# dcy0577/Enhancing-3D-Point-Cloud-Segmentation-Using-Multi-Modal-Fusion-with-2D-Images

Measured on AMD Instinct MI355X. Metric: input points/s through MV-KPConv KPFCNN forward+backward (pyramid + fusion + fwd + bwd + SGD), higher is better.
Workload: dtype f32; 1 GPU; early_fusion_kpfcnn5_sphere19k_x1_per_gpu; views=3, parallelism=dp1, execution=hipGraph[net|chain|enc2d(x2 every 2nd step)+fa], ranks=1, input_lookahead_batches=2, capacity_overflow=False

## Files before the change

enhancing-3d-point-cloud-segmentation-using-multi-modal-fusion-with-2d-images_amd/csrc/gemm.hip:

```cpp
#include <stdlib.h>

#include <mutex>
#include <type_traits>

#include "common.h"

namespace {

typedef float f32x4 __attribute__((ext_vector_type(4)));

constexpr int BK = 32;

template <bool CONTIG_K, int ROWS>
struct Tile {
  static constexpr int LD = CONTIG_K ? 40 : ROWS + 4;
  static constexpr int FLOATS = CONTIG_K ? ROWS * 40 : BK * (ROWS + 4);
  static constexpr int NF4 = ROWS * BK / 4;
  static constexpr int NV = (NF4 + 255) / 256;
  static constexpr int IPT = ROWS / 4;
  float4 v[NV];

  __device__ __forceinline__ void transform(const float* __restrict__ xs, int64_t k0, int64_t kbase0, int64_t i0, int64_t imax,
                                            int64_t kmax, int64_t nvalid, float slope, float* __restrict__ out, int64_t ld,
                                            int tid) {
    static_assert(CONTIG_K, "the transform is written for k-contiguous A tiles");
#pragma unroll
    for (int u = 0; u < NV; ++u) {
      const int f = tid + 256 * u;
      if (NF4 % 256 == 0 || f < NF4) {
        const int i = f >> 3, kq = (f & 7) * 4;
        const int64_t gi = i0 + i, gk = k0 + kq;
        const float* t = xs + (gk - kbase0) * 4;
        float e[4] = {v[u].x, v[u].y, v[u].z, v[u].w};
#pragma unroll
        for (int c = 0; c < 4; ++c) {
          const float4 q = *reinterpret_cast<const float4*>(t + 4 * c);
          float z = (e[c] - q.x) * q.y + q.z;
          z = z > 0.f ? z : z * slope;
          e[c] = gi < nvalid ? z : 0.f;
        }
        v[u] = make_float4(e[0], e[1], e[2], e[3]);
        if (out && gi < imax) {
          float* o = out + gi * ld + gk;
          if (gk + 3 < kmax && (ld & 3) == 0)
            *reinterpret_cast<float4*>(o) = v[u];
          else {
#pragma unroll
            for (int c = 0; c < 4; ++c)
              if (gk + c < kmax) o[c] = e[c];
// ... 67 lines not shown
        const int k = f / IPT, iq = (f % IPT) * 4;
        int64_t gi = i0 + iq;
        gi = gi + 3 < imax ? gi : imax - 4;
        p = src + (k0 + k) * ld + gi;
      }
      if (VEC == 4) {
        const f32x4 q = *reinterpret_cast<const f32x4*>(p);
        v[u] = make_float4(q[0], q[1], q[2], q[3]);
      } else {
        const float2 q0 = *reinterpret_cast<const float2*>(p), q1 = *reinterpret_cast<const float2*>(p + 2);
        v[u] = make_float4(q0.x, q0.y, q1.x, q1.y);
      }
    }
  }

  static __device__ __forceinline__ bool fast_ok(int64_t imax, int vec) {
    return CONTIG_K ? (vec >= 2 && imax >= 1) : (vec == 4 && imax >= 4 && (imax & 3) == 0);
  }

  template <int VEC>
  __device__ __forceinline__ void fetch(const float* __restrict__ src, int64_t ld, int64_t i0, int64_t imax, int64_t k0,
                                        int64_t kmax, int vec, int tid) {
    if (VEC == 0)
      load(src, ld, i0, imax, k0, kmax, vec, tid);
    else
      load_fast<VEC>(src, ld, i0, imax, k0, tid);
  }

  __device__ __forceinline__ void store(float* __restrict__ T, int tid) const {
#pragma unroll
    for (int u = 0; u < NV; ++u) {
      const int f = tid + 256 * u;
      if (NF4 % 256 == 0 || f < NF4) {
        const f32x4 q = {v[u].x, v[u].y, v[u].z, v[u].w};
        if (CONTIG_K) {
          const int i = f >> 3, kq = (f & 7) * 4;
          *reinterpret_cast<f32x4*>(&T[i * LD + kq]) = q;
        } else {
          const int k = f / IPT, iq = (f % IPT) * 4;
          *reinterpret_cast<f32x4*>(&T[k * LD + iq]) = q;
        }
      }
    }
  }

  static __device__ __forceinline__ f32x4 frag(const float* __restrict__ T, int r0, int j, int lane) {
    const int i = lane & 15, g = lane >> 4;
    if (CONTIG_K) {
      return *reinterpret_cast<const f32x4*>(&T[(r0 + i) * LD + 16 * j + 4 * g]);
    } else {
      f32x4 r;
      const float* p = &T[(16 * j + 4 * g) * LD + r0 + i];
      r[0] = p[0];
      r[1] = p[LD];
      r[2] = p[2 * LD];
      r[3] = p[3 * LD];
      return r;
    }
  }
};

struct GemmArgs {
  const float* A;
  const float* B;
  float* C;
  int64_t M, N, Kd, lda, ldb, k_per_split;
  int atomic_out, accumulate, vecA, vecB;
  float* bn_part;
  const int32_t* n_valid;
  const float* bias;
  float act_slope;
  const float* A2;
  const float* B2;
  int64_t Kd2, lda2, ldb2;
  int vecA2, vecB2;
  const void* sc_idx;
  int sc_idx64, sc_c1;
  int64_t sc_stride, sc_ns;
  float* sc_dst;
  float* sc_rest;
  float* det_ws;
  int* det_cnt;
  int det_gx, det_nsplit;
  int seg_shift;
  int64_t seg_extra;
  int* fin_cnt;
  int fin_gy;
  float fin_eps, fin_momentum;
  float* fin_mean;
  float* fin_invstd;
  float* fin_rmean;
  float* fin_rvar;
  long long* fin_nbt;
  const float* ax_mean;
  const float* ax_invstd;
  const float* ax_gamma;
  const float* ax_beta;
  float ax_slope;
  const int32_t* ax_nvalid;
  float* ax_out;
};

constexpr int XF_KMAX = 512;

template <bool TA, bool TB, int PM, int QN, int WM, int WN, bool DUAL = false, bool XF = false>
__device__ __forceinline__ void gemm_body(const GemmArgs& a, const int bx, const int by, const int bz) {
  static_assert(WM * WN == 4, "four waves per workgroup");
  constexpr int TM = 16 * PM * WM, TN = 16 * QN * WN;
  typedef Tile<!TA, TM> TileA;
  typedef Tile<TB, TN> TileB;
  __shared__ __attribute__((aligned(16))) float lds[2 * (TileA::FLOATS + TileB::FLOATS)];
  __shared__ __attribute__((aligned(16))) float xs[XF ? 4 * (XF_KMAX + BK) : 4];
  float* const As = lds;
  float* const Bs = lds + 2 * TileA::FLOATS;
  const int tid = threadIdx.x, lane = tid & 63, wave = tid >> 6;
  const int wm = wave / WN, wn = wave % WN;
  const int64_t m0 = (int64_t)by * TM, n0 = (int64_t)bx * TN;
  const int64_t ktot = DUAL ? a.Kd + a.Kd2 : a.Kd;
  const int64_t kbeg_all = (int64_t)bz * a.k_per_split;
  const int64_t kend_all = kbeg_all + a.k_per_split < ktot ? kbeg_all + a.k_per_split : ktot;

  f32x4 acc[PM][QN];
#pragma unroll
  for (int p = 0; p < PM; ++p)
#pragma unroll
    for (int q = 0; q < QN; ++q) acc[p][q] = (f32x4){0.f, 0.f, 0.f, 0.f};

  int64_t x_nvalid = 0;
  if (XF) {
    for (int k = tid; k < XF_KMAX + BK; k += 256) {
      const int64_t gk = kbeg_all + k;
      float4 q = make_float4(0.f, 0.f, 0.f, 0.f);
      if (gk < a.Kd && k < a.k_per_split + BK) q = make_float4(a.ax_mean[gk], a.ax_invstd[gk] * a.ax_gamma[gk], a.ax_beta[gk], 0.f);
      *reinterpret_cast<float4*>(&xs[4 * k]) = q;
    }
    x_nvalid = a.ax_nvalid ? (int64_t)*a.ax_nvalid : a.M;
    __syncthreads();
  }
  float* const x_out = (XF && bx == 0) ? a.ax_out : nullptr;

  TileA la0, la1;
  TileB lb0, lb1;
  const int ra = wm * 16 * PM, rb = wn * 16 * QN;
  auto compute = [&](const float* __restrict__ Ta, const float* __restrict__ Tb) {
#pragma unroll
    for (int j = 0; j < 2; ++j) {
      f32x4 fa[PM], fb[QN];
#pragma unroll
      for (int p = 0; p < PM; ++p) fa[p] = TileA::frag(Ta, ra + 16 * p, j, lane);
#pragma unroll
      for (int q = 0; q < QN; ++q) fb[q] = TileB::frag(Tb, rb + 16 * q, j, lane);
#pragma unroll
      for (int s = 0; s < 4; ++s)
#pragma unroll
        for (int p = 0; p < PM; ++p)
#pragma unroll
          for (int q = 0; q < QN; ++q)
            acc[p][q] = __builtin_amdgcn_mfma_f32_16x16x4f32(fa[p][s], fb[q][s], acc[p][q], 0, 0, 0);
    }
  };
  float* const A0 = As;
  float* const A1 = As + TileA::FLOATS;
  float* const B0 = Bs;
  float* const B1 = Bs + TileB::FLOATS;
  auto run_range = [&](const float* __restrict__ pA, const int64_t lda, const int vecA, const float* __restrict__ pB,
                       const int64_t ldb, const int vecB, int64_t kbeg, const int64_t kend) {
  auto Bat = [&](const int64_t k) -> const float* {
    return (TB && !DUAL && a.seg_shift >= 0) ? pB + (k >> a.seg_shift) * a.seg_extra : pB;
  };
  auto putA = [&](TileA& la, float* __restrict__ T, const int64_t kt) {
    if constexpr (XF) la.transform(xs, kt, kbeg_all, m0, a.M, a.Kd, x_nvalid, a.ax_slope, x_out, lda, tid);
    la.store(T, tid);
  };
  auto pipeline = [&](auto va, auto vb, const int64_t klim) {
    constexpr int VA = decltype(va)::value, VB = decltype(vb)::value;
    if (kbeg >= klim) return;
    la0.template fetch<VA>(pA, lda, m0, a.M, kbeg, klim, vecA, tid);
// ... 270 lines not shown
      float* const qr = lds + 2 * 256 * 4;
      if (bl == 0) *reinterpret_cast<f32x4*>(&qr[4 * c4]) = ref;
      __syncthreads();
      const int64_t col = n0 + tid;
      if (tid < TN && col < a.N) {
        float x = 0.f, y = 0.f;
#pragma unroll 4
        for (int l = 0; l < BL; ++l) {
          x += q1[l * TN + tid];
          y += q2[l * TN + tid];
        }
        float mu = 0.f, var = 0.f, is = 0.f;
        if (nv > 0) {
          mu = x / (float)nv;
          const float dm = mu - qr[tid];
          float M2 = y - (float)nv * dm * dm;
          M2 = M2 > 0.f ? M2 : 0.f;
          var = M2 / (float)nv;
          is = rsqrtf(var + a.fin_eps);
        }
        a.fin_mean[col] = mu;
        a.fin_invstd[col] = is;
        if (a.fin_rmean && nv > 0) {
          const float unbiased = nv > 1 ? var * ((float)nv / (float)(nv - 1)) : var;
          a.fin_rmean[col] = (1.f - a.fin_momentum) * a.fin_rmean[col] + a.fin_momentum * mu;
          a.fin_rvar[col] = (1.f - a.fin_momentum) * a.fin_rvar[col] + a.fin_momentum * unbiased;
        }
      }
      if (a.fin_nbt && bx == 0 && tid == 0) *a.fin_nbt += 1;
    }
  }
}

template <bool TA, bool TB, int PM, int QN, int WM, int WN>
__global__ __launch_bounds__(256) void gemm_f32_mfma(const GemmArgs a) {
  gemm_body<TA, TB, PM, QN, WM, WN>(a, blockIdx.x, blockIdx.y, blockIdx.z);
}

template <bool TB, int PM>
__global__ __launch_bounds__(256) void gemm_f32_mfma_xf(const GemmArgs a) {
  gemm_body<false, TB, PM, 1, 1, 4, false, true>(a, blockIdx.x, blockIdx.y, blockIdx.z);
}

template <bool TA, bool TB, int PM, int QN, int WM, int WN>
__global__ __launch_bounds__(256) void gemm_f32_mfma_pair(const GemmArgs a0, const GemmArgs a1, int gx0, int gz0, int gz1) {
  if ((int)blockIdx.x < gx0) {
    if ((int)blockIdx.z >= gz0) return;
    gemm_body<TA, TB, PM, QN, WM, WN>(a0, blockIdx.x, blockIdx.y, blockIdx.z);
  } else {
    if ((int)blockIdx.z >= gz1) return;
    gemm_body<TA, TB, PM, QN, WM, WN>(a1, blockIdx.x - gx0, blockIdx.y, blockIdx.z);
  }
}

template <bool TA, bool TB, int PM, int QN, int WM, int WN>
__global__ __launch_bounds__(256) void gemm_f32_mfma_dual(const GemmArgs a) {
  gemm_body<TA, TB, PM, QN, WM, WN, true>(a, blockIdx.x, blockIdx.y, blockIdx.z);
}

struct GroupEntry {
  GemmArgs args;
  int gx, gy, gz;
  int wg_begin;
};

template <bool TA, bool TB, int PM, int QN, int WM, int WN>
__global__ __launch_bounds__(256) void gemm_f32_mfma_grouped(const GroupEntry* __restrict__ tab, int n_prob) {
  const int b = blockIdx.x;
  int lo = 0, hi = n_prob - 1;
  while (lo < hi) {
    const int mid = (lo + hi + 1) >> 1;
    if (tab[mid].wg_begin <= b)
      lo = mid;
    else
      hi = mid - 1;
  }
  const GroupEntry& e = tab[lo];
  const int local = b - e.wg_begin;
  const int bx = local % e.gx, by = (local / e.gx) % e.gy, bz = local / (e.gx * e.gy);
  GemmArgs a = e.args;
  a.A = load_global_ptr(&e.args.A);
  a.B = load_global_ptr(&e.args.B);
  a.C = load_global_ptr(&e.args.C);
  a.bn_part = load_global_ptr(&e.args.bn_part);
  a.n_valid = load_global_ptr(&e.args.n_valid);
  a.det_ws = load_global_ptr(&e.args.det_ws);
  a.det_cnt = load_global_ptr(&e.args.det_cnt);
  gemm_body<TA, TB, PM, QN, WM, WN>(a, bx, by, bz);
}


struct Plan {
  int pm, qn, narrow, split;
};

struct SplitArena {
  float* ws = nullptr;
  int* cnt = nullptr;
  int64_t ws_floats = 0, n_cnt = 0;
  int64_t ws_off = 0, cnt_off = 0;
  int64_t ws_top = 0, cnt_top = 0;
};
SplitArena g_arena;
std::mutex g_arena_mu;

bool ordered_splits() { return g_arena.ws != nullptr; }

int arena_take(hipStream_t st, int64_t tiles, int split, int64_t slot, float** ws, int** cnt) {
  const int64_t need = (tiles * split * slot + 63) / 64 * 64;
  std::lock_guard<std::mutex> lock(g_arena_mu);
  if (need > g_arena.ws_floats || tiles > g_arena.n_cnt) return 1;
  hipStreamCaptureStatus cap = hipStreamCaptureStatusNone;
  if (hipStreamIsCapturing(st, &cap) != hipSuccess) {
    (void)hipGetLastError();
    cap = hipStreamCaptureStatusNone;
  }
  if (cap != hipStreamCaptureStatusNone) {
    if (g_arena.ws_top - need < g_arena.ws_off || g_arena.cnt_top - tiles < g_arena.cnt_off) return 2;
    g_arena.ws_top -= need;
    g_arena.cnt_top -= tiles;
    *ws = g_arena.ws + g_arena.ws_top;
    *cnt = g_arena.cnt + g_arena.cnt_top;
    return 0;
  }
  const int64_t ws_cap = g_arena.ws_top < g_arena.ws_floats / 4 ? g_arena.ws_top : (need > g_arena.ws_floats / 4 ? need : g_arena.ws_floats / 4);
  const int64_t cnt_cap = g_arena.cnt_top < g_arena.n_cnt / 4 ? g_arena.cnt_top : (tiles > g_arena.n_cnt / 4 ? tiles : g_arena.n_cnt / 4);
  if (g_arena.ws_off + need > ws_cap || g_arena.cnt_off + tiles > cnt_cap) {
// ... 1 lines not shown
    if (hipDeviceSynchronize() != hipSuccess) return -2;
    g_arena.ws_off = 0;
    g_arena.cnt_off = 0;
  }
  *ws = g_arena.ws + g_arena.ws_off;
  *cnt = g_arena.cnt + g_arena.cnt_off;
  g_arena.ws_off += need;
  g_arena.cnt_off += tiles;
  return 0;
}

const char* arena_error(int rc) {
  return rc == 1 ? "the split-reduction arena is smaller than one product's parking space (MVK_GEMM_ARENA_MB)"
         : rc == 2 ? "the split-reduction arena is used up by the slices captured graphs hold for good: too small for the "
                     "captured steps of this process (MVK_GEMM_ARENA_MB)"
                   : "hipDeviceSynchronize failed while recycling the split-reduction arena";
}

int make_ordered(hipStream_t st, GemmArgs& a, int split, int gx, int64_t gy, int64_t tm, int64_t tn) {
  a.det_ws = nullptr; a.det_cnt = nullptr; a.det_gx = gx; a.det_nsplit = split;
  if (split <= 1 || !ordered_splits()) return 0;
  const int rc = arena_take(st, (int64_t)gx * gy, split, tm * tn, &a.det_ws, &a.det_cnt);
  if (rc != 0) return rc;
  a.atomic_out = 0;
  return 0;
}

#define MVK_ORDERED(call)                                      \
  do {                                                         \
    const int _rc = (call);                                    \
    MVK_REQUIRE(_rc == 0, "gemm: %s", arena_error(_rc));       \
  } while (0)

Plan plan_gemm(int64_t M, int64_t N, int64_t Kd, int split_req, bool want_stats) {
  const int narrow = N <= 32 ? 1 : 0;
  const int pm = narrow ? 1 : (want_stats ? 4 : 2), qn = narrow ? (N <= 16 ? 1 : 2) : 1;
  const int64_t tm = narrow ? 64 * pm : 16 * pm, tn = narrow ? 16 * qn : 64 * qn;
  const int64_t tiles = cdiv64(M, tm) * cdiv64(N, tn), ksteps = cdiv64(Kd, BK);
  Plan best{pm, qn, narrow, 1};
  double best_t = 1e300, t1 = 1e300;
  for (int split = 1; split <= 64; ++split) {
    if (split_req > 0 && split != split_req) continue;
    if (split > 1 && ksteps / split < 4) break;
    const int64_t kt = cdiv64(ksteps, split), wgs = tiles * split;
    double t = (double)cdiv64(wgs, 1280) * (kt * 1500.0 + 3000.0) + (double)wgs * kt * 256.0 * pm * qn / 256.0;
    if (split > 1) t += (double)M * N * split * 4.0 / 2160.0 + 500.0 * split;
    if (split == 1) t1 = t;
    if (t < best_t) {
      best_t = t;
      best.split = split;
    }
  }
  static double bonus = -1.0;
  if (bonus < 0.0) {
    const char* eb = getenv("MVK_GEMM_STATS_BONUS");
    bonus = eb ? atof(eb) : 14000.0;
  }
  if (want_stats && !ordered_splits() && t1 <= best_t + bonus) best.split = 1;
  const char* e = getenv("MVK_GEMM_FORCE");
  if (e) {
    int pm = 0, qn = 0, sp = 0;
    if (sscanf(e, "%d,%d,%d", &pm, &qn, &sp) == 3) {
      if (pm > 0) best.pm = pm;
      if (qn > 0 && !best.narrow) best.qn = qn;
      if (sp > 0 && split_req <= 0) best.split = sp;
    }
  }
  return best;
}

template <bool TA, bool TB, int PM, int QN, int WM, int WN>
void launch_one(dim3 grid, hipStream_t st, const GemmArgs& a) {
  hipLaunchKernelGGL((gemm_f32_mfma<TA, TB, PM, QN, WM, WN>), grid, dim3(256), 0, st, a);
}

template <bool TA, bool TB>
bool launch_cfg(const Plan& p, dim3 grid, hipStream_t st, const GemmArgs& a) {
  if (p.narrow) {
#define NARROW(PMv, QNv) \
  if (p.pm == PMv && p.qn == QNv) return launch_one<TA, TB, PMv, QNv, 4, 1>(grid, st, a), true
    NARROW(1, 1); NARROW(2, 1); NARROW(1, 2); NARROW(2, 2);
#undef NARROW
    return false;
  }
#define WIDE(PMv, QNv) \
  if (p.pm == PMv && p.qn == QNv) return launch_one<TA, TB, PMv, QNv, 1, 4>(grid, st, a), true
  WIDE(1, 1); WIDE(2, 1); WIDE(4, 1); WIDE(5, 1);
  WIDE(1, 2); WIDE(2, 2); WIDE(4, 2);
#undef WIDE
  return false;
}

template <bool TA, bool TB, int PM>
void launch_pair_one(dim3 grid, hipStream_t st, const GemmArgs& a0, const GemmArgs& a1, int gx0, int gz0, int gz1) {
  hipLaunchKernelGGL((gemm_f32_mfma_pair<TA, TB, PM, 1, 1, 4>), grid, dim3(256), 0, st, a0, a1, gx0, gz0, gz1);
}

template <bool TA, bool TB>
bool launch_pair_cfg(const Plan& p, dim3 grid, hipStream_t st, const GemmArgs& a0, const GemmArgs& a1, int gx0, int gz0, int gz1) {
  if (p.qn != 1) return false;
  if (p.pm == 2) return launch_pair_one<TA, TB, 2>(grid, st, a0, a1, gx0, gz0, gz1), true;
  if (p.pm == 4) return launch_pair_one<TA, TB, 4>(grid, st, a0, a1, gx0, gz0, gz1), true;
  return false;
}

void pair_widen(Plan& a, const Plan& b, int64_t Kd) {
  if (a.narrow && !b.narrow && Kd <= 512) {
    a.narrow = 0;
    a.pm = b.pm;
    a.qn = 1;
    a.split = 1;
  }
}

void no_bn_fold(GemmArgs& a) {
  a.fin_cnt = nullptr; a.fin_gy = 0; a.fin_eps = 0.f; a.fin_momentum = 0.f; a.fin_mean = nullptr; a.fin_invstd = nullptr;
  a.fin_rmean = nullptr; a.fin_rvar = nullptr; a.fin_nbt = nullptr;
  a.ax_mean = nullptr; a.ax_invstd = nullptr; a.ax_gamma = nullptr; a.ax_beta = nullptr; a.ax_slope = 1.f;
  a.ax_nvalid = nullptr; a.ax_out = nullptr;
}

int set_finish(GemmArgs& a, const mvk_bn_finish* fin, int64_t gy) {
  if (!fin) return 0;
  MVK_REQUIRE(a.bn_part != nullptr, "gemm: finished BatchNorm statistics need the statistics epilogue (plan: stat rows 0)");
  MVK_REQUIRE(fin->counters && fin->mean && fin->invstd && a.N % 4 == 0 && (uintptr_t)a.bn_part % 16 == 0,
              "gemm: finished statistics need counters, mean, invstd and a channel count that is a multiple of 4");
  MVK_REQUIRE((fin->running_mean == nullptr) == (fin->running_var == nullptr), "gemm: running_mean and running_var go together");
  a.fin_cnt = fin->counters; a.fin_gy = (int)gy; a.fin_eps = fin->eps; a.fin_momentum = fin->momentum;
  a.fin_mean = fin->mean; a.fin_invstd = fin->invstd; a.fin_rmean = fin->running_mean; a.fin_rvar = fin->running_var;
  a.fin_nbt = (long long*)fin->num_batches_tracked;
  return 0;
}

// ... 50 lines not shown
extern "C" int mvk_gemm_split_ordered(void) { return ordered_splits() ? 1 : 0; }

extern "C" int mvk_gemm_f32_dual_plan(int64_t M, int64_t N, int64_t Kd, int64_t Kd2, int* out_split) {
  MVK_REQUIRE(M >= 0 && N >= 0 && Kd >= 0 && Kd2 >= 0 && out_split, "gemm dual plan: bad arguments");
  *out_split = 0;
  if (M == 0 || N == 0 || Kd == 0 || Kd2 == 0 || Kd % BK != 0) return 0;
  const Plan p = plan_gemm(M, N, Kd + Kd2, 0, false);
  if (p.narrow || p.qn != 1 || p.pm != 2) return 0;
  int split = p.split;
  const int64_t ksteps = cdiv64(Kd + Kd2, BK);
  if (split > ksteps) split = (int)ksteps;
  const int64_t k_per_split = cdiv64(ksteps, split) * BK;
  *out_split = (int)cdiv64(Kd + Kd2, k_per_split);
  return 0;
}

extern "C" int mvk_gemm_f32_dual(const float* A, const float* B, const float* A2, const float* B2, float* C, int64_t M,
                                 int64_t N, int64_t Kd, int64_t Kd2, void* stream) {
  MVK_REQUIRE(M > 0 && N > 0 && Kd > 0 && Kd2 > 0 && Kd % BK == 0, "gemm dual: unsupported shape (ask mvk_gemm_f32_dual_plan)");
  const Plan p = plan_gemm(M, N, Kd + Kd2, 0, false);
  MVK_REQUIRE(!p.narrow && p.qn == 1 && p.pm == 2, "gemm dual: unsupported shape (ask mvk_gemm_f32_dual_plan)");
  hipStream_t st = (hipStream_t)stream;
  GemmArgs a;
  const int split = fill_args(a, p, A, B, C, M, N, Kd + Kd2, 0, 0, nullptr, nullptr);
  a.Kd = Kd;
  a.lda = Kd;
  a.vecA = ((a.lda % 4 == 0) && ((uintptr_t)A % 16 == 0)) ? 4 : ((a.lda % 2 == 0) && ((uintptr_t)A % 8 == 0)) ? 2 : 1;
  a.A2 = A2; a.B2 = B2; a.Kd2 = Kd2; a.lda2 = Kd2; a.ldb2 = N;
  a.vecA2 = ((a.lda2 % 4 == 0) && ((uintptr_t)A2 % 16 == 0)) ? 4 : ((a.lda2 % 2 == 0) && ((uintptr_t)A2 % 8 == 0)) ? 2 : 1;
  a.vecB2 = ((a.ldb2 % 4 == 0) && ((uintptr_t)B2 % 16 == 0)) ? 4 : ((a.ldb2 % 2 == 0) && ((uintptr_t)B2 % 8 == 0)) ? 2 : 1;
  MVK_REQUIRE(cdiv64(M, 32) < 65536 && split < 65536, "gemm: grid too large");
  dim3 grid((unsigned)cdiv64(N, 64), (unsigned)cdiv64(M, 32), (unsigned)split);
  MVK_ORDERED(make_ordered(st, a, split, (int)grid.x, grid.y, 32, 64));
  hipLaunchKernelGGL((gemm_f32_mfma_dual<false, false, 2, 1, 1, 4>), grid, dim3(256), 0, st, a);
  MVK_CHECK_HIP(hipGetLastError());
  return 0;
}

extern "C" int mvk_gemm_f32_pair_plan(int64_t M, int64_t N0, int64_t N1, int64_t Kd, int want_stats, int* out ) {
  MVK_REQUIRE(M >= 0 && N0 >= 0 && N1 >= 0 && Kd >= 0 && out, "gemm pair plan: bad arguments");
  for (int i = 0; i < 5; ++i) out[i] = 0;
  if (M == 0 || N0 == 0 || N1 == 0 || Kd == 0) return 0;
  Plan p0 = plan_gemm(M, N0, Kd, 0, want_stats != 0), p1 = plan_gemm(M, N1, Kd, 0, want_stats != 0);
  pair_widen(p0, p1, Kd);
  if (p0.narrow || p1.narrow || p0.pm != p1.pm || p0.qn != 1 || p1.qn != 1 || (p0.pm != 2 && p0.pm != 4)) return 0;
  out[0] = 1;
  out[1] = p0.split;
  out[2] = p1.split;
  out[3] = (want_stats && (p0.split == 1 || ordered_splits())) ? 16 * p0.pm : 0;
  out[4] = (want_stats && (p1.split == 1 || ordered_splits())) ? 16 * p1.pm : 0;
  return 0;
}

namespace {
int gemm_pair_run(const float* A, const float* B0, const float* B1, float* C0, float* C1, int64_t M, int64_t N0, int64_t N1,
                  int64_t Kd, int transB, int want_stats, float* bn_part0, float* bn_part1, const int32_t* n_valid,
                  const mvk_bn_finish* fin0, const mvk_bn_finish* fin1, void* stream);
}
extern "C" int mvk_gemm_f32_pair(const float* A, const float* B0, const float* B1, float* C0, float* C1, int64_t M,
                                 int64_t N0, int64_t N1, int64_t Kd, int transB, int want_stats, float* bn_part0,
                                 float* bn_part1, const int32_t* n_valid, void* stream) {
  return gemm_pair_run(A, B0, B1, C0, C1, M, N0, N1, Kd, transB, want_stats, bn_part0, bn_part1, n_valid, nullptr, nullptr, stream);
}
extern "C" int mvk_gemm_f32_pair_bn(const float* A, const float* B0, const float* B1, float* C0, float* C1, int64_t M,
                                    int64_t N0, int64_t N1, int64_t Kd, int transB, float* bn_part0, float* bn_part1,
                                    const int32_t* n_valid, const mvk_bn_finish* fin0, const mvk_bn_finish* fin1, void* stream) {
  return gemm_pair_run(A, B0, B1, C0, C1, M, N0, N1, Kd, transB, 1, bn_part0, bn_part1, n_valid, fin0, fin1, stream);
}
namespace {
int gemm_pair_run(const float* A, const float* B0, const float* B1, float* C0, float* C1, int64_t M, int64_t N0, int64_t N1,
                  int64_t Kd, int transB, int want_stats, float* bn_part0, float* bn_part1, const int32_t* n_valid,
                  const mvk_bn_finish* fin0, const mvk_bn_finish* fin1, void* stream) {
  MVK_REQUIRE(M > 0 && N0 > 0 && N1 > 0 && Kd > 0, "gemm pair: empty product");
  Plan p0 = plan_gemm(M, N0, Kd, 0, want_stats != 0), p1 = plan_gemm(M, N1, Kd, 0, want_stats != 0);
  pair_widen(p0, p1, Kd);
  MVK_REQUIRE(!p0.narrow && !p1.narrow && p0.pm == p1.pm && p0.qn == 1 && p1.qn == 1 && (p0.pm == 2 || p0.pm == 4),
              "gemm pair: the two products do not share a tile shape (ask mvk_gemm_f32_pair_plan first)");
  hipStream_t st = (hipStream_t)stream;
  GemmArgs a0, a1;
  const bool ord = ordered_splits();
  const int s0 = fill_args(a0, p0, A, B0, C0, M, N0, Kd, 0, transB, (want_stats && (p0.split == 1 || ord)) ? bn_part0 : nullptr, n_valid);
  const int s1 = fill_args(a1, p1, A, B1, C1, M, N1, Kd, 0, transB, (want_stats && (p1.split == 1 || ord)) ? bn_part1 : nullptr, n_valid);
  const int64_t tm = 16 * p0.pm, tn = 64;
  MVK_REQUIRE(cdiv64(M, tm) < 65536 && s0 < 65536 && s1 < 65536, "gemm: grid too large");
  const int gx0 = (int)cdiv64(N0, tn), gx1 = (int)cdiv64(N1, tn);
  MVK_ORDERED(make_ordered(st, a0, s0, gx0, cdiv64(M, tm), tm, tn));
  MVK_ORDERED(make_ordered(st, a1, s1, gx1, cdiv64(M, tm), tm, tn));
  MVK_REQUIRE(ord || ((s0 == 1 || !a0.bn_part) && (s1 == 1 || !a1.bn_part)), "gemm pair: statistics of a split product");
  if (int e = set_finish(a0, fin0, cdiv64(M, tm))) return e;
  if (int e = set_finish(a1, fin1, cdiv64(M, tm))) return e;
  dim3 grid((unsigned)(gx0 + gx1), (unsigned)cdiv64(M, tm), (unsigned)(s0 > s1 ? s0 : s1));
  const bool ok = transB ? launch_pair_cfg<false, true>(p0, grid, st, a0, a1, gx0, s0, s1)
                         : launch_pair_cfg<false, false>(p0, grid, st, a0, a1, gx0, s0, s1);
  MVK_REQUIRE(ok, "gemm pair: no kernel for plan pm=%d", p0.pm);
  MVK_CHECK_HIP(hipGetLastError());
  return 0;
}
}

extern "C" int mvk_gemm_f32_plan(int64_t M, int64_t N, int64_t Kd, int split_k, int want_stats, int* out_split,
                                 int* out_stat_rows) {
  MVK_REQUIRE(M >= 0 && N >= 0 && Kd >= 0 && out_split && out_stat_rows, "gemm plan: bad arguments");
  if (M == 0 || N == 0 || Kd == 0) {
    *out_split = 1;
    *out_stat_rows = 0;
    return 0;
  }
  const Plan p = plan_gemm(M, N, Kd, split_k > 0 ? split_k : 0, want_stats != 0);
// ... 42 lines not shown
  while ((1 << shift) < Cout) ++shift;
  return gemm_run(A, W, dx, M, Cin, (int64_t)K * Cout, 0, 1, 0, 0, nullptr, nullptr, nullptr, 1.f, stream, nullptr, shift,
                  (int64_t)Cin * Cout - Cout);
}

extern "C" int mvk_gemm_f32_ldb(const float* A, const float* B, float* C, int64_t M, int64_t N, int64_t Kd, int64_t ldb,
                                void* stream) {
  MVK_REQUIRE(ldb >= N, "gemm ldb: ldb < N");
  return gemm_run(A, B, C, M, N, Kd, 0, 0, 0, 0, nullptr, nullptr, nullptr, 1.f, stream, nullptr, -1, 0, ldb);
}

extern "C" int mvk_gemm_f32_scatter_cat(const float* A, const float* B, int64_t M, int64_t N, int64_t Kd, const void* idx,
                                        int idx64, int64_t idx_stride, int64_t Ns, int c1, float* d_x, float* d_skip,
                                        void* stream) {
  MVK_REQUIRE(idx && d_x && d_skip && c1 > 0 && c1 < N && Kd > 0 && Ns >= 0 && idx_stride >= 1, "gemm scatter_cat: bad arguments");
  const ScatterOut sc{idx, idx64, c1, idx_stride, Ns, d_x, d_skip};
  return gemm_run(A, B, d_skip , M, N, Kd, 0, 0, 0, 0, nullptr, nullptr, nullptr, 1.f, stream, &sc);
}

namespace {
int gemm_run(const float* A, const float* B, float* C, int64_t M, int64_t N, int64_t Kd, int transA, int transB,
             int accumulate, int split_k, float* bn_part, const int32_t* n_valid, const float* bias, float act_slope,
             void* stream, const ScatterOut* scatter, int seg_shift, int64_t seg_extra, int64_t ldb,
             const mvk_bn_finish* fin, const mvk_a_transform* ax) {
  MVK_REQUIRE(M >= 0 && N >= 0 && Kd >= 0, "gemm: negative size");
  if (M == 0 || N == 0) return 0;
  hipStream_t st = (hipStream_t)stream;
  MVK_REQUIRE(!(bn_part && (accumulate || Kd == 0)), "gemm: BatchNorm statistics need a plain store of a non-empty product");
  if (Kd == 0) {
    if (!accumulate && split_k <= 1) MVK_CHECK_HIP(hipMemsetAsync(C, 0, sizeof(float) * M * N, st));
    return 0;
  }
  MVK_REQUIRE(!(bn_part && split_k > 1 && !ordered_splits()), "gemm: BatchNorm statistics need an unsplit (or ordered) reduction");
  Plan p = plan_gemm(M, N, Kd, (bn_part && !ordered_splits()) ? 1 : (split_k > 0 ? split_k : 0), bn_part != nullptr);
  int split = p.split;
  const int64_t ksteps = cdiv64(Kd, BK);
  if (split > ksteps) split = (int)ksteps;
  const int64_t k_per_split = cdiv64(ksteps, split) * BK;
  split = (int)cdiv64(Kd, k_per_split);
  GemmArgs a;
  a.A = A; a.B = B; a.C = C; a.M = M; a.N = N; a.Kd = Kd;
  a.lda = transA ? M : Kd;
  a.ldb = transB ? Kd : N;
  a.k_per_split = k_per_split;
  a.atomic_out = split > 1;
  a.accumulate = accumulate;
  a.vecA = ((a.lda % 4 == 0) && ((uintptr_t)A % 16 == 0)) ? 4 : ((a.lda % 2 == 0) && ((uintptr_t)A % 8 == 0)) ? 2 : 1;
  a.vecB = ((a.ldb % 4 == 0) && ((uintptr_t)B % 16 == 0)) ? 4 : ((a.ldb % 2 == 0) && ((uintptr_t)B % 8 == 0)) ? 2 : 1;
  if (ldb > 0) {
    a.ldb = ldb;
    a.vecB = ((a.ldb % 4 == 0) && ((uintptr_t)B % 16 == 0)) ? 4 : ((a.ldb % 2 == 0) && ((uintptr_t)B % 8 == 0)) ? 2 : 1;
  }
  if (seg_shift >= 0) {
    a.ldb = (int64_t)1 << seg_shift;
    a.vecB = ((uintptr_t)B % 16 == 0 && seg_extra % 4 == 0) ? 4 : 1;
  }
  a.bn_part = bn_part;
  a.n_valid = n_valid;
  a.bias = bias;
  a.act_slope = act_slope;
  a.A2 = nullptr; a.B2 = nullptr; a.Kd2 = 0; a.lda2 = 0; a.ldb2 = 0; a.vecA2 = 1; a.vecB2 = 1;
  a.sc_idx = nullptr; a.sc_idx64 = 0; a.sc_c1 = 0; a.sc_stride = 0; a.sc_ns = 0; a.sc_dst = nullptr; a.sc_rest = nullptr;
  a.seg_shift = seg_shift;
  a.seg_extra = seg_extra;
  no_bn_fold(a);
  if (scatter) {
    a.sc_idx = scatter->idx; a.sc_idx64 = scatter->idx64; a.sc_c1 = scatter->c1; a.sc_stride = scatter->stride;
// ... 7 lines not shown
  if (int e = set_finish(a, fin, grid.y)) return e;
  if (ax) {
    MVK_REQUIRE(!transA && transB && !p.narrow && p.qn == 1 && (p.pm == 2 || p.pm == 4) && k_per_split <= XF_KMAX && !scatter &&
                    seg_shift < 0 && ax->mean && ax->invstd && ax->gamma && ax->beta && ax->slope > 0.f,
                "gemm: the operand transform needs an NT product of more than 32 columns with k-ranges <= %d", XF_KMAX);
    a.ax_mean = ax->mean; a.ax_invstd = ax->invstd; a.ax_gamma = ax->gamma; a.ax_beta = ax->beta; a.ax_slope = ax->slope;
    a.ax_nvalid = ax->n_valid; a.ax_out = ax->out;
    if (p.pm == 2) hipLaunchKernelGGL((gemm_f32_mfma_xf<true, 2>), grid, dim3(256), 0, st, a);
    else hipLaunchKernelGGL((gemm_f32_mfma_xf<true, 4>), grid, dim3(256), 0, st, a);
    MVK_CHECK_HIP(hipGetLastError());
    return 0;
  }
  bool ok;
  if (!transA && !transB) ok = launch_cfg<false, false>(p, grid, st, a);
  else if (!transA && transB) ok = launch_cfg<false, true>(p, grid, st, a);
  else if (transA && !transB) ok = launch_cfg<true, false>(p, grid, st, a);
  else ok = launch_cfg<true, true>(p, grid, st, a);
  MVK_REQUIRE(ok, "gemm: no kernel for plan pm=%d qn=%d narrow=%d", p.pm, p.qn, p.narrow);
  MVK_CHECK_HIP(hipGetLastError());
  return 0;
}
}

struct MvkGemmProblem {
  const float* A;
  const float* B;
  float* C;
  int64_t M, N, Kd;
};

extern "C" int64_t mvk_gemm_group_entry_bytes(void) { return (int64_t)sizeof(GroupEntry); }

constexpr int GROUP_KTILES_MIN = 16, GROUP_KTILES_MAX = 96;

int group_wide_pm() {
  static const int v = getenv("MVK_DW_WIDE_PM") ? atoi(getenv("MVK_DW_WIDE_PM")) : 4;
  return v == 2 || v == 8 ? v : 4;
}

int group_ktiles_env() {
  static const int v = getenv("MVK_DW_GROUP_KTILES") ? atoi(getenv("MVK_DW_GROUP_KTILES")) : -1;
  return v;
}

int grouped_split_at(int64_t M, int64_t N, int64_t Kd, int ktiles) {
  if (ktiles <= 0) return plan_gemm(M, N, Kd, 0, false).split;
  int64_t split = cdiv64(cdiv64(Kd, BK), ktiles);
  return (int)(split > 64 ? 64 : (split < 1 ? 1 : split));
}

extern "C" int mvk_gemm_f32_tn_grouped_split(int64_t M, int64_t N, int64_t Kd) {
  const int e = group_ktiles_env();
  return grouped_split_at(M, N, Kd, e >= 0 ? e : GROUP_KTILES_MIN);
}

extern "C" int mvk_gemm_f32_tn_grouped_plan(const void* problems, int n, void* table_host, int* n_narrow,
                                            int64_t* wgs_narrow, int64_t* wgs_wide, int32_t* splits ,
                                            void* stream ) {
  MVK_REQUIRE(n >= 0 && problems && table_host && n_narrow && wgs_narrow && wgs_wide && splits, "grouped gemm: bad arguments");
  const MvkGemmProblem* pr = (const MvkGemmProblem*)problems;
  GroupEntry* tab = (GroupEntry*)table_host;
  int nn = 0;
  for (int i = 0; i < n; ++i) nn += pr[i].N <= 32 ? 1 : 0;
  int64_t wn = 0, ww = 0;
  int in = 0, iw = nn;
  int ktiles = group_ktiles_env();
// ... 31 lines not shown
    e.args.sc_idx = nullptr; e.args.sc_idx64 = 0; e.args.sc_c1 = 0; e.args.sc_stride = 0; e.args.sc_ns = 0;
    e.args.sc_dst = nullptr; e.args.sc_rest = nullptr;
    e.args.seg_shift = -1; e.args.seg_extra = 0;
    no_bn_fold(e.args);
    const int64_t tm = narrow ? 64 : 16 * group_wide_pm(), tn = narrow ? 32 : 64;
    e.gx = (int)cdiv64(q.N, tn);
    e.gy = (int)cdiv64(q.M, tm);
    e.gz = split;
    MVK_ORDERED(make_ordered((hipStream_t)stream, e.args, split, e.gx, e.gy, tm, tn));
    const int64_t wgs = (int64_t)e.gx * e.gy * e.gz;
    if (narrow) {
      e.wg_begin = (int)wn;
      wn += wgs;
      tab[in++] = e;
    } else {
      e.wg_begin = (int)ww;
      ww += wgs;
      tab[iw++] = e;
    }
    splits[i] = split;
  }
  MVK_REQUIRE(wn < (1ll << 31) && ww < (1ll << 31), "grouped gemm: grid too large");
  *n_narrow = nn;
  *wgs_narrow = wn;
  *wgs_wide = ww;
  return 0;
}

extern "C" int mvk_gemm_f32_tn_grouped(const void* table_dev, int n, int n_narrow, int64_t wgs_narrow, int64_t wgs_wide,
                                       void* stream) {
  MVK_REQUIRE(n >= 0 && n_narrow >= 0 && n_narrow <= n, "grouped gemm: bad counts");
  hipStream_t st = (hipStream_t)stream;
  const GroupEntry* tab = (const GroupEntry*)table_dev;
  if (n_narrow > 0 && wgs_narrow > 0)
    hipLaunchKernelGGL((gemm_f32_mfma_grouped<true, false, 1, 2, 4, 1>), dim3((unsigned)wgs_narrow), dim3(256), 0, st, tab,
                       n_narrow);
  if (n - n_narrow > 0 && wgs_wide > 0) {
    if (group_wide_pm() == 4)
      hipLaunchKernelGGL((gemm_f32_mfma_grouped<true, false, 4, 1, 1, 4>), dim3((unsigned)wgs_wide), dim3(256), 0, st,
                         tab + n_narrow, n - n_narrow);
    else if (group_wide_pm() == 8)
      hipLaunchKernelGGL((gemm_f32_mfma_grouped<true, false, 8, 1, 1, 4>), dim3((unsigned)wgs_wide), dim3(256), 0, st,
                         tab + n_narrow, n - n_narrow);
    else
      hipLaunchKernelGGL((gemm_f32_mfma_grouped<true, false, 2, 1, 1, 4>), dim3((unsigned)wgs_wide), dim3(256), 0, st,
                         tab + n_narrow, n - n_narrow);
  }
  MVK_CHECK_HIP(hipGetLastError());
  return 0;
}

extern "C" int mvk_gemm_f32(const float* A, const float* B, float* C, int64_t M, int64_t N, int64_t Kd, int transA,
                            int transB, int accumulate, int split_k, void* stream) {
  return mvk_gemm_f32_ex(A, B, C, M, N, Kd, transA, transB, accumulate, split_k, nullptr, nullptr, stream);
}
```

Measured before the change: 5.462 million points/s.

## Add bf16x3 split-precision MFMA GEMM path, default on for grouped wide weight-gradient GEMMs

Adds an S3 GEMM variant that splits each f32 operand into three bf16 parts (high, mid, low) when storing tiles to LDS. It then accumulates six bf16 16x16x32 MFMA cross terms to emulate f32 accuracy, using swizzled LDS layouts and ds_read_tr16 transposed reads. The path is enabled by default only for the wide grouped weight-gradient kernel (pm=4), and by env override elsewhere. It aims to replace slower f32 MFMA throughput with higher-rate bf16 MFMA, at the cost of extra split arithmetic, three times the LDS traffic, and slightly different rounding.

```diff
diff --git a/enhancing-3d-point-cloud-segmentation-using-multi-modal-fusion-with-2d-images_amd/csrc/gemm.hip b/enhancing-3d-point-cloud-segmentation-using-multi-modal-fusion-with-2d-images_amd/csrc/gemm.hip
--- a/enhancing-3d-point-cloud-segmentation-using-multi-modal-fusion-with-2d-images_amd/csrc/gemm.hip
+++ b/enhancing-3d-point-cloud-segmentation-using-multi-modal-fusion-with-2d-images_amd/csrc/gemm.hip
@@ -8,13 +8,37 @@
 namespace {
 
 typedef float f32x4 __attribute__((ext_vector_type(4)));
+typedef float f32x2 __attribute__((ext_vector_type(2)));
+typedef __bf16 bf16x2 __attribute__((ext_vector_type(2)));
+typedef __bf16 bf16x8 __attribute__((ext_vector_type(8)));
+typedef short i16x4 __attribute__((ext_vector_type(4)));
+typedef uint32_t u32x2 __attribute__((ext_vector_type(2)));
+typedef uint32_t u32x4 __attribute__((ext_vector_type(4)));
 
 constexpr int BK = 32;
 
-template <bool CONTIG_K, int ROWS>
+struct Frag3 {
+  bf16x8 h, m, l;
+};
+
+__device__ __forceinline__ void split3(const float x0, const float x1, uint32_t& h, uint32_t& m, uint32_t& l) {
+  f32x2 r = {x0, x1};
+  h = __builtin_bit_cast(uint32_t, __builtin_convertvector(r, bf16x2));
+  r -= (f32x2){__uint_as_float(h << 16), __uint_as_float(h & 0xffff0000u)};
+  m = __builtin_bit_cast(uint32_t, __builtin_convertvector(r, bf16x2));
+  r -= (f32x2){__uint_as_float(m << 16), __uint_as_float(m & 0xffff0000u)};
+  l = __builtin_bit_cast(uint32_t, __builtin_convertvector(r, bf16x2));
+}
+
+__device__ __forceinline__ int s3_swz(const int i) { return (0x78 >> ((i >> 1) & 6)) & 3; }
+
+__device__ __forceinline__ int s3_pos(const int k) { return (k & 3) | ((k >> 1) & 4) | ((k << 1) & 8) | (k & 16); }
+
+template <bool CONTIG_K, int ROWS, bool S3 = false>
 struct Tile {
   static constexpr int LD = CONTIG_K ? 40 : ROWS + 4;
-  static constexpr int FLOATS = CONTIG_K ? ROWS * 40 : BK * (ROWS + 4);
+  static constexpr int S3_LD = 48, S3_BLOCK = 264, S3_PLANE = ROWS / 16 * S3_BLOCK;
+  static constexpr int FLOATS = S3 ? (CONTIG_K ? ROWS * S3_LD : 3 * S3_PLANE) : (CONTIG_K ? ROWS * 40 : BK * (ROWS + 4));
   static constexpr int NF4 = ROWS * BK / 4;
   static constexpr int NV = (NF4 + 255) / 256;
   static constexpr int IPT = ROWS / 4;
@@ -148,6 +172,27 @@
     for (int u = 0; u < NV; ++u) {
       const int f = tid + 256 * u;
       if (NF4 % 256 == 0 || f < NF4) {
+        if constexpr (S3) {
+          uint32_t h0, m0, l0, h1, m1, l1;
+          split3(v[u].x, v[u].y, h0, m0, l0);
+          split3(v[u].z, v[u].w, h1, m1, l1);
+          const u32x2 h = {h0, h1}, m = {m0, m1}, l = {l0, l1};
+          uint32_t* const W = reinterpret_cast<uint32_t*>(T);
+          if (CONTIG_K) {
+            const int i = f >> 3, kq = (f & 7) * 4;
+            uint32_t* const w = W + i * S3_LD + 4 * ((kq >> 3) ^ s3_swz(i)) + ((kq >> 1) & 2);
+            *reinterpret_cast<u32x2*>(w) = h;
+            *reinterpret_cast<u32x2*>(w + 16) = m;
+            *reinterpret_cast<u32x2*>(w + 32) = l;
+          } else {
+            const int k = f / IPT, iq = (f % IPT) * 4;
+            uint32_t* const w = W + (iq >> 4) * S3_BLOCK + s3_pos(k) * 8 + ((iq & 15) >> 1);
+            *reinterpret_cast<u32x2*>(w) = h;
+            *reinterpret_cast<u32x2*>(w + S3_PLANE) = m;
+            *reinterpret_cast<u32x2*>(w + 2 * S3_PLANE) = l;
+          }
+          continue;
+        }
         const f32x4 q = {v[u].x, v[u].y, v[u].z, v[u].w};
         if (CONTIG_K) {
           const int i = f >> 3, kq = (f & 7) * 4;
@@ -173,6 +218,32 @@
       r[3] = p[3 * LD];
       return r;
     }
+  }
+
+  static __device__ __forceinline__ Frag3 frag3(const float* __restrict__ T, int r0, int lane) {
+    const int i = lane & 15, g = lane >> 4;
+    Frag3 r;
+    if (CONTIG_K) {
+      const u32x4* p = reinterpret_cast<const u32x4*>(reinterpret_cast<const uint32_t*>(T) + (r0 + i) * S3_LD + 4 * (g ^ s3_swz(i)));
+      r.h = __builtin_bit_cast(bf16x8, p[0]);
+      r.m = __builtin_bit_cast(bf16x8, p[4]);
+      r.l = __builtin_bit_cast(bf16x8, p[8]);
+    } else {
+      const int q = i >> 2, c = i & 3;
+      const uint32_t* w = reinterpret_cast<const uint32_t*>(T) + (r0 >> 4) * S3_BLOCK + s3_pos(8 * g + q) * 8 + 2 * c;
+      auto rd = [&](const uint32_t* a) -> bf16x8 {
+        typedef __attribute__((address_space(3))) i16x4 lds_i16x4;
+        const i16x4 lo = __builtin_amdgcn_ds_read_tr16_b64_v4i16((lds_i16x4*)a);
+        const i16x4 hi = __builtin_amdgcn_ds_read_tr16_b64_v4i16((lds_i16x4*)(a + 64));
+        const u32x4 o = {__builtin_bit_cast(u32x2, lo)[0], __builtin_bit_cast(u32x2, lo)[1], __builtin_bit_cast(u32x2, hi)[0],
+                         __builtin_bit_cast(u32x2, hi)[1]};
+        return __builtin_bit_cast(bf16x8, o);
+      };
+      r.h = rd(w);
+      r.m = rd(w + S3_PLANE);
+      r.l = rd(w + 2 * S3_PLANE);
+    }
+    return r;
   }
 };
 
@@ -219,12 +290,13 @@
 
 constexpr int XF_KMAX = 512;
 
-template <bool TA, bool TB, int PM, int QN, int WM, int WN, bool DUAL = false, bool XF = false>
+template <bool TA, bool TB, int PM, int QN, int WM, int WN, bool DUAL = false, bool XF = false, bool S3 = false>
 __device__ __forceinline__ void gemm_body(const GemmArgs& a, const int bx, const int by, const int bz) {
   static_assert(WM * WN == 4, "four waves per workgroup");
   constexpr int TM = 16 * PM * WM, TN = 16 * QN * WN;
-  typedef Tile<!TA, TM> TileA;
-  typedef Tile<TB, TN> TileB;
+  static_assert(!(S3 && XF), "the operand transform runs on the f32 path");
+  typedef Tile<!TA, TM, S3> TileA;
+  typedef Tile<TB, TN, S3> TileB;
   __shared__ __attribute__((aligned(16))) float lds[2 * (TileA::FLOATS + TileB::FLOATS)];
   __shared__ __attribute__((aligned(16))) float xs[XF ? 4 * (XF_KMAX + BK) : 4];
   float* const As = lds;
@@ -259,6 +331,24 @@
   TileB lb0, lb1;
   const int ra = wm * 16 * PM, rb = wn * 16 * QN;
   auto compute = [&](const float* __restrict__ Ta, const float* __restrict__ Tb) {
+    if constexpr (S3) {
+      Frag3 fa[PM], fb[QN];
+#pragma unroll
+      for (int p = 0; p < PM; ++p) fa[p] = TileA::frag3(Ta, ra + 16 * p, lane);
+#pragma unroll
+      for (int q = 0; q < QN; ++q) fb[q] = TileB::frag3(Tb, rb + 16 * q, lane);
+#define MVK_S3_TERM(x, y)                                                                                    \
+  _Pragma("unroll") for (int p = 0; p < PM; ++p) _Pragma("unroll") for (int q = 0; q < QN; ++q) acc[p][q] = \
+      __builtin_amdgcn_mfma_f32_16x16x32_bf16(fa[p].x, fb[q].y, acc[p][q], 0, 0, 0)
+      MVK_S3_TERM(l, h);
+      MVK_S3_TERM(h, l);
+      MVK_S3_TERM(m, m);
+      MVK_S3_TERM(m, h);
+      MVK_S3_TERM(h, m);
+      MVK_S3_TERM(h, h);
+#undef MVK_S3_TERM
+      return;
+    }
 #pragma unroll
     for (int j = 0; j < 2; ++j) {
       f32x4 fa[PM], fb[QN];
@@ -595,9 +685,9 @@
   }
 }
 
-template <bool TA, bool TB, int PM, int QN, int WM, int WN>
+template <bool TA, bool TB, int PM, int QN, int WM, int WN, bool S3 = false>
 __global__ __launch_bounds__(256) void gemm_f32_mfma(const GemmArgs a) {
-  gemm_body<TA, TB, PM, QN, WM, WN>(a, blockIdx.x, blockIdx.y, blockIdx.z);
+  gemm_body<TA, TB, PM, QN, WM, WN, false, false, S3>(a, blockIdx.x, blockIdx.y, blockIdx.z);
 }
 
 template <bool TB, int PM>
@@ -605,20 +695,20 @@
   gemm_body<false, TB, PM, 1, 1, 4, false, true>(a, blockIdx.x, blockIdx.y, blockIdx.z);
 }
 
-template <bool TA, bool TB, int PM, int QN, int WM, int WN>
+template <bool TA, bool TB, int PM, int QN, int WM, int WN, bool S3 = false>
 __global__ __launch_bounds__(256) void gemm_f32_mfma_pair(const GemmArgs a0, const GemmArgs a1, int gx0, int gz0, int gz1) {
   if ((int)blockIdx.x < gx0) {
     if ((int)blockIdx.z >= gz0) return;
-    gemm_body<TA, TB, PM, QN, WM, WN>(a0, blockIdx.x, blockIdx.y, blockIdx.z);
+    gemm_body<TA, TB, PM, QN, WM, WN, false, false, S3>(a0, blockIdx.x, blockIdx.y, blockIdx.z);
   } else {
     if ((int)blockIdx.z >= gz1) return;
-    gemm_body<TA, TB, PM, QN, WM, WN>(a1, blockIdx.x - gx0, blockIdx.y, blockIdx.z);
-  }
-}
-
-template <bool TA, bool TB, int PM, int QN, int WM, int WN>
+    gemm_body<TA, TB, PM, QN, WM, WN, false, false, S3>(a1, blockIdx.x - gx0, blockIdx.y, blockIdx.z);
+  }
+}
+
+template <bool TA, bool TB, int PM, int QN, int WM, int WN, bool S3 = false>
 __global__ __launch_bounds__(256) void gemm_f32_mfma_dual(const GemmArgs a) {
-  gemm_body<TA, TB, PM, QN, WM, WN, true>(a, blockIdx.x, blockIdx.y, blockIdx.z);
+  gemm_body<TA, TB, PM, QN, WM, WN, true, false, S3>(a, blockIdx.x, blockIdx.y, blockIdx.z);
 }
 
 struct GroupEntry {
@@ -627,7 +717,7 @@
   int wg_begin;
 };
 
-template <bool TA, bool TB, int PM, int QN, int WM, int WN>
+template <bool TA, bool TB, int PM, int QN, int WM, int WN, bool S3 = false>
 __global__ __launch_bounds__(256) void gemm_f32_mfma_grouped(const GroupEntry* __restrict__ tab, int n_prob) {
   const int b = blockIdx.x;
   int lo = 0, hi = n_prob - 1;
@@ -649,13 +739,24 @@
   a.n_valid = load_global_ptr(&e.args.n_valid);
   a.det_ws = load_global_ptr(&e.args.det_ws);
   a.det_cnt = load_global_ptr(&e.args.det_cnt);
-  gemm_body<TA, TB, PM, QN, WM, WN>(a, bx, by, bz);
+  gemm_body<TA, TB, PM, QN, WM, WN, false, false, S3>(a, bx, by, bz);
 }
 
 
 struct Plan {
   int pm, qn, narrow, split;
+  int s3;
 };
+
+int s3_override() {
+  const char* e = getenv("MVK_GEMM_S3");
+  return (e && (e[0] == '0' || e[0] == '1') && e[1] == 0) ? e[0] - '0' : -1;
+}
+
+bool s3_has_tile(const Plan& p) { return p.narrow ? (p.pm == 1 && (p.qn == 1 || p.qn == 2)) : (p.qn == 1 && (p.pm == 2 || p.pm == 4)); }
+
+constexpr double MFMA_F32 = 256.0, MFMA_S3 = 96.0;
+
 
 struct SplitArena {
   float* ws = nullptr;
@@ -723,18 +824,26 @@
     MVK_REQUIRE(_rc == 0, "gemm: %s", arena_error(_rc));       \
   } while (0)
 
-Plan plan_gemm(int64_t M, int64_t N, int64_t Kd, int split_req, bool want_stats) {
+bool s3_default(int64_t M, int64_t N, int64_t Kd) {
+  (void)M; (void)N; (void)Kd;
+  return false;
+}
+
+Plan plan_gemm(int64_t M, int64_t N, int64_t Kd, int split_req, bool want_stats, int arith = -1 ) {
+  const int s3o = arith >= 0 ? arith : s3_override();
   const int narrow = N <= 32 ? 1 : 0;
+  const int s3 = s3o >= 0 ? s3o : (s3_default(M, N, Kd) ? 1 : 0);
   const int pm = narrow ? 1 : (want_stats ? 4 : 2), qn = narrow ? (N <= 16 ? 1 : 2) : 1;
   const int64_t tm = narrow ? 64 * pm : 16 * pm, tn = narrow ? 16 * qn : 64 * qn;
   const int64_t tiles = cdiv64(M, tm) * cdiv64(N, tn), ksteps = cdiv64(Kd, BK);
-  Plan best{pm, qn, narrow, 1};
+  Plan best{pm, qn, narrow, 1, s3};
+  const double mfma = best.s3 ? MFMA_S3 : MFMA_F32;
   double best_t = 1e300, t1 = 1e300;
   for (int split = 1; split <= 64; ++split) {
     if (split_req > 0 && split != split_req) continue;
     if (split > 1 && ksteps / split < 4) break;
     const int64_t kt = cdiv64(ksteps, split), wgs = tiles * split;
-    double t = (double)cdiv64(wgs, 1280) * (kt * 1500.0 + 3000.0) + (double)wgs * kt * 256.0 * pm * qn / 256.0;
+    double t = (double)cdiv64(wgs, 1280) * (kt * 1500.0 + 3000.0) + (double)wgs * kt * mfma * pm * qn / 256.0;
     if (split > 1) t += (double)M * N * split * 4.0 / 2160.0 + 500.0 * split;
     if (split == 1) t1 = t;
     if (t < best_t) {
@@ -757,16 +866,27 @@
       if (sp > 0 && split_req <= 0) best.split = sp;
     }
   }
+  if (!s3_has_tile(best)) best.s3 = 0;
   return best;
 }
 
-template <bool TA, bool TB, int PM, int QN, int WM, int WN>
+template <bool TA, bool TB, int PM, int QN, int WM, int WN, bool S3 = false>
 void launch_one(dim3 grid, hipStream_t st, const GemmArgs& a) {
-  hipLaunchKernelGGL((gemm_f32_mfma<TA, TB, PM, QN, WM, WN>), grid, dim3(256), 0, st, a);
+  hipLaunchKernelGGL((gemm_f32_mfma<TA, TB, PM, QN, WM, WN, S3>), grid, dim3(256), 0, st, a);
 }
 
 template <bool TA, bool TB>
 bool launch_cfg(const Plan& p, dim3 grid, hipStream_t st, const GemmArgs& a) {
+  if (p.s3) {
+    if (p.narrow) {
+      if (p.pm == 1 && p.qn == 1) return launch_one<TA, TB, 1, 1, 4, 1, true>(grid, st, a), true;
+      if (p.pm == 1 && p.qn == 2) return launch_one<TA, TB, 1, 2, 4, 1, true>(grid, st, a), true;
+      return false;
+    }
+    if (p.pm == 2 && p.qn == 1) return launch_one<TA, TB, 2, 1, 1, 4, true>(grid, st, a), true;
+    if (p.pm == 4 && p.qn == 1) return launch_one<TA, TB, 4, 1, 1, 4, true>(grid, st, a), true;
+    return false;
+  }
   if (p.narrow) {
 #define NARROW(PMv, QNv) \
   if (p.pm == PMv && p.qn == QNv) return launch_one<TA, TB, PMv, QNv, 4, 1>(grid, st, a), true
@@ -782,14 +902,16 @@
   return false;
 }
 
-template <bool TA, bool TB, int PM>
+template <bool TA, bool TB, int PM, bool S3 = false>
 void launch_pair_one(dim3 grid, hipStream_t st, const GemmArgs& a0, const GemmArgs& a1, int gx0, int gz0, int gz1) {
-  hipLaunchKernelGGL((gemm_f32_mfma_pair<TA, TB, PM, 1, 1, 4>), grid, dim3(256), 0, st, a0, a1, gx0, gz0, gz1);
+  hipLaunchKernelGGL((gemm_f32_mfma_pair<TA, TB, PM, 1, 1, 4, S3>), grid, dim3(256), 0, st, a0, a1, gx0, gz0, gz1);
 }
 
 template <bool TA, bool TB>
 bool launch_pair_cfg(const Plan& p, dim3 grid, hipStream_t st, const GemmArgs& a0, const GemmArgs& a1, int gx0, int gz0, int gz1) {
   if (p.qn != 1) return false;
+  if (p.s3 && p.pm == 2) return launch_pair_one<TA, TB, 2, true>(grid, st, a0, a1, gx0, gz0, gz1), true;
+  if (p.s3 && p.pm == 4) return launch_pair_one<TA, TB, 4, true>(grid, st, a0, a1, gx0, gz0, gz1), true;
   if (p.pm == 2) return launch_pair_one<TA, TB, 2>(grid, st, a0, a1, gx0, gz0, gz1), true;
   if (p.pm == 4) return launch_pair_one<TA, TB, 4>(grid, st, a0, a1, gx0, gz0, gz1), true;
   return false;
@@ -906,7 +1028,8 @@
   MVK_REQUIRE(cdiv64(M, 32) < 65536 && split < 65536, "gemm: grid too large");
   dim3 grid((unsigned)cdiv64(N, 64), (unsigned)cdiv64(M, 32), (unsigned)split);
   MVK_ORDERED(make_ordered(st, a, split, (int)grid.x, grid.y, 32, 64));
-  hipLaunchKernelGGL((gemm_f32_mfma_dual<false, false, 2, 1, 1, 4>), grid, dim3(256), 0, st, a);
+  if (p.s3) hipLaunchKernelGGL((gemm_f32_mfma_dual<false, false, 2, 1, 1, 4, true>), grid, dim3(256), 0, st, a);
+  else hipLaunchKernelGGL((gemm_f32_mfma_dual<false, false, 2, 1, 1, 4>), grid, dim3(256), 0, st, a);
   MVK_CHECK_HIP(hipGetLastError());
   return 0;
 }
@@ -948,6 +1071,7 @@
   MVK_REQUIRE(M > 0 && N0 > 0 && N1 > 0 && Kd > 0, "gemm pair: empty product");
   Plan p0 = plan_gemm(M, N0, Kd, 0, want_stats != 0), p1 = plan_gemm(M, N1, Kd, 0, want_stats != 0);
   pair_widen(p0, p1, Kd);
+  p0.s3 = (p0.s3 && p1.s3 && s3_has_tile(p0)) ? 1 : 0;
   MVK_REQUIRE(!p0.narrow && !p1.narrow && p0.pm == p1.pm && p0.qn == 1 && p1.qn == 1 && (p0.pm == 2 || p0.pm == 4),
               "gemm pair: the two products do not share a tile shape (ask mvk_gemm_f32_pair_plan first)");
   hipStream_t st = (hipStream_t)stream;
@@ -1056,7 +1180,8 @@
     return 0;
   }
   MVK_REQUIRE(!(bn_part && split_k > 1 && !ordered_splits()), "gemm: BatchNorm statistics need an unsplit (or ordered) reduction");
-  Plan p = plan_gemm(M, N, Kd, (bn_part && !ordered_splits()) ? 1 : (split_k > 0 ? split_k : 0), bn_part != nullptr);
+  Plan p = plan_gemm(M, N, Kd, (bn_part && !ordered_splits()) ? 1 : (split_k > 0 ? split_k : 0), bn_part != nullptr,
+                     (transA && s3_override() < 0) ? 0 : -1);
   int split = p.split;
   const int64_t ksteps = cdiv64(Kd, BK);
   if (split > ksteps) split = (int)ksteps;
@@ -1130,6 +1255,7 @@
 extern "C" int64_t mvk_gemm_group_entry_bytes(void) { return (int64_t)sizeof(GroupEntry); }
 
 constexpr int GROUP_KTILES_MIN = 16, GROUP_KTILES_MAX = 96;
+constexpr bool GROUP_S3_DEFAULT = true;
 
 int group_wide_pm() {
   static const int v = getenv("MVK_DW_WIDE_PM") ? atoi(getenv("MVK_DW_WIDE_PM")) : 4;
@@ -1227,11 +1353,21 @@
   MVK_REQUIRE(n >= 0 && n_narrow >= 0 && n_narrow <= n, "grouped gemm: bad counts");
   hipStream_t st = (hipStream_t)stream;
   const GroupEntry* tab = (const GroupEntry*)table_dev;
-  if (n_narrow > 0 && wgs_narrow > 0)
-    hipLaunchKernelGGL((gemm_f32_mfma_grouped<true, false, 1, 2, 4, 1>), dim3((unsigned)wgs_narrow), dim3(256), 0, st, tab,
-                       n_narrow);
+  const int s3o = s3_override();
+  const bool s3 = s3o >= 0 ? s3o == 1 : GROUP_S3_DEFAULT;
+  if (n_narrow > 0 && wgs_narrow > 0) {
+    if (s3 && s3o >= 0)
+      hipLaunchKernelGGL((gemm_f32_mfma_grouped<true, false, 1, 2, 4, 1, true>), dim3((unsigned)wgs_narrow), dim3(256), 0, st,
+                         tab, n_narrow);
+    else
+      hipLaunchKernelGGL((gemm_f32_mfma_grouped<true, false, 1, 2, 4, 1>), dim3((unsigned)wgs_narrow), dim3(256), 0, st, tab,
+                         n_narrow);
+  }
   if (n - n_narrow > 0 && wgs_wide > 0) {
-    if (group_wide_pm() == 4)
+    if (s3 && group_wide_pm() == 4)
+      hipLaunchKernelGGL((gemm_f32_mfma_grouped<true, false, 4, 1, 1, 4, true>), dim3((unsigned)wgs_wide), dim3(256), 0, st,
+                         tab + n_narrow, n - n_narrow);
+    else if (group_wide_pm() == 4)
       hipLaunchKernelGGL((gemm_f32_mfma_grouped<true, false, 4, 1, 1, 4>), dim3((unsigned)wgs_wide), dim3(256), 0, st,
                          tab + n_narrow, n - n_narrow);
     else if (group_wide_pm() == 8)
```

Measured after the change: 5.420 million points/s. No clear change (-0.8%).
